# ARM-software/astc-encoder

Hardware: AMD Instinct MI355X
Metric: Mtexels/s + PSNR-dB, 8192x8192 RGBA8 LDR 6x6 -medium (higher is better)
Workload: dtype f32

## Files before the change

astc-encoder_amd/csrc/wave_partition.h:

```cpp
#pragma once
#include "wave_ctx.h"

namespace astcd { inline namespace ASTC_VARIANT {

struct PartScratch {
	uint64_t bitmaps[4];
	uint16_t mscount[64];
	int      best_count;
	int      best[MAX_PARTITIONING_CANDIDATES];
	int      n;
	int      lim;
	uint8_t  pad[256 - 32 - 128 - 4 - 32 - 8];
	WV_FN uint16_t* ordering() { return reinterpret_cast<uint16_t*>(reinterpret_cast<uint8_t*>(this) + 256); }
	WV_FN float* uncor_err() { return reinterpret_cast<float*>(reinterpret_cast<uint8_t*>(this) + 256 + n * 2); }
	WV_FN float* samec_err() { return uncor_err() + lim; }
	WV_FN uint8_t* mismatch() { return reinterpret_cast<uint8_t*>(samec_err() + lim); }
};
static_assert(sizeof(PartScratch) == 256, "PartScratch header");

WV_FN int mismatch2(const uint64_t* a, const uint64_t* b)
{
	int v1 = popcount64(a[0] ^ b[0]) + popcount64(a[1] ^ b[1]);
	int v2 = popcount64(a[0] ^ b[1]) + popcount64(a[1] ^ b[0]);
	return i_min(v1, v2) / 2;
}

WV_FN int mismatch3(const uint64_t* a, const uint64_t* b)
{
	int p00 = popcount64(a[0] ^ b[0]), p01 = popcount64(a[0] ^ b[1]), p02 = popcount64(a[0] ^ b[2]);
	int p10 = popcount64(a[1] ^ b[0]), p11 = popcount64(a[1] ^ b[1]), p12 = popcount64(a[1] ^ b[2]);
	int p20 = popcount64(a[2] ^ b[0]), p21 = popcount64(a[2] ^ b[1]), p22 = popcount64(a[2] ^ b[2]);
	int v0 = i_min(p11 + p22, p12 + p21) + p00;
	int v1 = i_min(p10 + p22, p12 + p20) + p01;
	int v2 = i_min(p10 + p21, p11 + p20) + p02;
	return i_min(i_min(v0, v1), v2) / 2;
}

WV_FN int mismatch4(const uint64_t* a, const uint64_t* b)
{
	int p[4][4];
	for (int i = 0; i < 4; i++) for (int j = 0; j < 4; j++) p[i][j] = popcount64(a[i] ^ b[j]);
	int mx23 = i_min(p[2][2] + p[3][3], p[2][3] + p[3][2]);
	int mx13 = i_min(p[2][1] + p[3][3], p[2][3] + p[3][1]);
	int mx12 = i_min(p[2][1] + p[3][2], p[2][2] + p[3][1]);
	int mx03 = i_min(p[2][0] + p[3][3], p[2][3] + p[3][0]);
	int mx02 = i_min(p[2][0] + p[3][2], p[2][2] + p[3][0]);
	int mx01 = i_min(p[2][1] + p[3][0], p[2][0] + p[3][1]);
	int v0 = p[0][0] + i_min(i_min(p[1][1] + mx23, p[1][2] + mx13), p[1][3] + mx12);
	int v1 = p[0][1] + i_min(i_min(p[1][0] + mx23, p[1][2] + mx03), p[1][3] + mx02);
	int v2 = p[0][2] + i_min(i_min(p[1][1] + mx03, p[1][0] + mx13), p[1][3] + mx01);
	int v3 = p[0][3] + i_min(i_min(p[1][1] + mx02, p[1][2] + mx01), p[1][0] + mx12);
	return i_min(i_min(v0, v1), i_min(v2, v3)) / 2;
}

WV_FN int kmeans_partition_ordering(const Ctx& c, int pc, PartScratch& ps)
{
	TrialInfo& tr = c.tr();
	const BlkInfo& blk = c.blk();
	const int T = c.T;
	float* dist = c.tsc_p(0);
	float* assign = c.tsc_p(1);
	const f4 cw = cw4_of(blk);
	float* centers = &tr.fbox[0];

	{
		int sample = 145897 % T;
		WV_ONE { for (int k = 0; k < 4; k++) centers[k] = c.data(k)[sample]; }
		WV_SYNC();
		int clusters_selected = 1;

		WV_FOR_T(i, T)
		{
			f4 color = mk4(c.data(0)[i], c.data(1)[i], c.data(2)[i], c.data(3)[i]);
			f4 diff = color - load4(centers);
			dist[i] = dot_s(diff * diff, cw);
		}
		WV_SYNC();

		const float cluster_cutoffs[9] = {
			0.626220f, 0.932770f, 0.275454f,
			0.318558f, 0.240113f, 0.009190f,
			0.347661f, 0.731960f, 0.156391f
		};
		int cutoff = (clusters_selected - 1) + 3 * (pc - 2);

		while (true)
		{
			float distance_sum = 0.0f;
			for (int i = 0; i < T; i++) distance_sum += dist[i];

			float summa = 0.0f;
			float distance_cutoff = distance_sum * cluster_cutoffs[cutoff++];
			sample = T;
			for (int i = 0; i < T; i++)
			{
				summa += dist[i];
				sample = (sample == T && summa >= distance_cutoff) ? i : sample;
			}
			sample = i_min(sample, T - 1);

			WV_SYNC();
			WV_ONE { for (int k = 0; k < 4; k++) centers[clusters_selected * 4 + k] = c.data(k)[sample]; }
			WV_SYNC();
			clusters_selected++;
			if (clusters_selected >= pc) break;

			WV_FOR_T(i, T)
			{
				f4 color = mk4(c.data(0)[i], c.data(1)[i], c.data(2)[i], c.data(3)[i]);
				f4 diff = color - load4(&centers[(clusters_selected - 1) * 4]);
				float distance = dot_s(diff * diff, cw);
				dist[i] = f_min(distance, dist[i]);
			}
			WV_SYNC();
		}
	}

	for (int iter = 0; iter < 3; iter++)
	{
		if (iter > 0)
		{
			WV_FOR64(k, pc * 4)
			{
				int p = k >> 2, ch = k & 3;
				const float* d = c.data(ch);
				float sum = 0.0f;
				int cnt = 0;
				for (int i = 0; i < T; i++)
				{
					const bool mine = (int)assign[i] == p;
					sum += mine ? d[i] : 0.0f;
					cnt += mine ? 1 : 0;
				}
				float scale = 1.0f / (float)cnt;
				tr.fbox[16 + k] = sum * scale;
			}
			WV_SYNC();
			WV_FOR64(k, pc * 4) { centers[k] = tr.fbox[16 + k]; }
			WV_SYNC();
		}

		WV_FOR_T(i, T)
		{
			float best_distance = 3.402823466e+38f;
			int best_partition = 0;
			f4 color = mk4(c.data(0)[i], c.data(1)[i], c.data(2)[i], c.data(3)[i]);
			for (int j = 0; j < pc; j++)
			{
				f4 diff = color - load4(&centers[j * 4]);
				float distance = dot_s(diff * diff, cw);
				if (distance < best_distance)
				{
					best_distance = distance;
					best_partition = j;
				}
			}
			assign[i] = (float)best_partition;
		}
		WV_SYNC();

		{
			int c0 = 0, c1 = 0, c2 = 0, c3 = 0;
#if WV_DEVICE
			for (int base = 0; base < T; base += 64)
			{
				const int i = base + WV_LANE;
				const int a = i < T ? (int)assign[i] : -1;
				c0 += __popcll(__ballot(a == 0)); c1 += __popcll(__ballot(a == 1));
				c2 += __popcll(__ballot(a == 2)); c3 += __popcll(__ballot(a == 3));
			}
#else
			for (int i = 0; i < T; i++)
			{
				int a = (int)assign[i];
				c0 += a == 0; c1 += a == 1; c2 += a == 2; c3 += a == 3;
			}
#endif
			bool any_empty = false;
			for (int i = 0; i < pc; i++) any_empty = any_empty || (i == 0 ? c0 : i == 1 ? c1 : i == 2 ? c2 : c3) == 0;
			if (any_empty)
			{
				WV_ONE
				{
					bool problem_case;
					do
					{
						problem_case = false;
						for (int i = 0; i < pc; i++)
						{
							int ci = i == 0 ? c0 : i == 1 ? c1 : i == 2 ? c2 : c3;
							if (ci == 0)
							{
								int a = (int)assign[i];
								c0 -= a == 0; c1 -= a == 1; c2 -= a == 2; c3 -= a == 3;
								c0 += i == 0; c1 += i == 1; c2 += i == 2; c3 += i == 3;
								assign[i] = (float)i;
								problem_case = true;
							}
						}
					} while (problem_case);
				}
				WV_SYNC();
			}
		}
	}

	const int texels_to_process = i_min(T, MAX_KMEANS_TEXELS);
	const uint8_t* km = c.table(c.root->off_kmeans_texels);
#if WV_DEVICE
	{
		const int a = WV_LANE < texels_to_process ? (int)assign[km[WV_LANE]] : -1;
		for (int p = 0; p < pc; p++)
		{
			const uint64_t bm = __ballot(a == p);
			WV_ONE { ps.bitmaps[p] = bm; }
		}
	}
#else
	WV_FOR64(p, pc)
	{
		uint64_t bm = 0;
		for (int i = 0; i < texels_to_process; i++)
		{
			if ((int)assign[km[i]] == p) bm |= 1ULL << i;
		}
		ps.bitmaps[p] = bm;
	}
#endif
	WV_SYNC();

	const int count = (int)c.root->partitioning_count_selected[pc - 1];
	const uint64_t* cov = reinterpret_cast<const uint64_t*>(c.table(c.root->off_coverage[pc - 1]));
	WV_FOR(i, count)
	{
		int m;
		if (pc == 2) m = mismatch2(ps.bitmaps, cov + i * 2);
		else if (pc == 3) m = mismatch3(ps.bitmaps, cov + i * 3);
		else m = mismatch4(ps.bitmaps, cov + i * 4);
		ps.mismatch()[i] = (uint8_t)m;
	}
	WV_SYNC();

#if WV_DEVICE
	{
		const int lane = WV_LANE;
		const uint8_t* mm = ps.mismatch();
		uint16_t* ord = ps.ordering();
		int* bins = &tr.ibox[0];
		bins[lane] = 0;
		WV_SYNC();
		auto same_key_lanes = [](int m, bool valid) -> unsigned long long
		{
			unsigned long long mask = __ballot(valid);
			#pragma unroll
			for (int k = 0; k < 6; k++)
			{
				const bool bit = ((m >> k) & 1) != 0;
				const unsigned long long with_bit = __ballot(bit);
				mask &= bit ? with_bit : ~with_bit;
			}
			return mask;
		};
		auto lanes_below = [](unsigned long long mask) -> int
		{
			return (int)__builtin_amdgcn_mbcnt_hi((uint32_t)(mask >> 32), __builtin_amdgcn_mbcnt_lo((uint32_t)mask, 0u));
		};
		for (int first = 0; first < count; first += 64)
		{
			const int i = first + lane;
			const bool valid = i < count;
			const int m = valid ? (int)mm[i] : 0;
			const unsigned long long same = same_key_lanes(m, valid);
			if (valid && lanes_below(same) == 0) bins[m] += (int)__popcll(same);
			WV_SYNC();
		}
		WV_SYNC();
		{
			const int hist = bins[lane];
			int base = hist;
			for (int d = 1; d < 64; d <<= 1)
			{
				int up = __shfl_up(base, d);
				if (lane >= d) base += up;
			}
			bins[lane] = base - hist;
		}
		WV_SYNC();
		for (int first = 0; first < count; first += 64)
		{
			const int i = first + lane;
			const bool valid = i < count;
			const int m = valid ? (int)mm[i] : 0;
			const unsigned long long same = same_key_lanes(m, valid);
			const int rank = lanes_below(same);
			const int start = bins[m];
			if (valid) ord[start + rank] = (uint16_t)i;
			if (valid && rank == 0) bins[m] = start + (int)__popcll(same);
			WV_SYNC();
		}
		(void)texels_to_process;
	}
#else
	WV_ONE
	{
		for (int i = 0; i < 64; i++) ps.mscount[i] = 0;
		for (int i = 0; i < count; i++) ps.mscount[ps.mismatch()[i]]++;
		uint16_t sum = 0;
		for (int i = 0; i < texels_to_process; i++)
		{
			uint16_t cnt = ps.mscount[i];
			ps.mscount[i] = sum;
			sum = (uint16_t)(sum + cnt);
		}
		for (int i = 0; i < count; i++)
		{
			unsigned int idx = ps.mscount[ps.mismatch()[i]]++;
			ps.ordering()[idx] = (uint16_t)i;
		}
	}
#endif
	WV_SYNC();
	return count;
}

template <bool USES_ALPHA>
WV_FN void score_partitioning(const Ctx& c, int pc, const PartView& pv, float weight_imprecision_estim, float& uncor_out, float& samec_out)
{
	const BlkInfo& blk = c.blk();
	const int T = c.T, Tp = c.Tp;
	constexpr int n = USES_ALPHA ? 4 : 3;

	float avg[4][4];
	{
		float rest[4];
		#pragma unroll
		for (int ch = 0; ch < 4; ch++) rest[ch] = blk.data_mean[ch] * (float)T;
		const uint32_t* ot4 = reinterpret_cast<const uint32_t*>(pv.of_texel);
		#pragma unroll
		for (int p = 0; p < 3; p++)
		{
			if (p >= pc - 1) break;
			float acc[4][4];
			#pragma unroll
			for (int ch = 0; ch < 4; ch++)
				#pragma unroll
				for (int l = 0; l < 4; l++) acc[ch][l] = 0.0f;
			#pragma nounroll
			for (int i = 0; i < Tp; i += 4)
			{
				const uint32_t ot = ot4[i >> 2];
				const float m0 = (int)(ot & 0xFF) == p ? 1.0f : 0.0f;
				const float m1 = (int)((ot >> 8) & 0xFF) == p ? 1.0f : 0.0f;
				const float m2 = (int)((ot >> 16) & 0xFF) == p ? 1.0f : 0.0f;
				const float m3 = (int)(ot >> 24) == p ? 1.0f : 0.0f;
				#pragma unroll
				for (int ch = 0; ch < 4; ch++)
				{
					if (ch >= n) break;
					const float* d = c.data(ch) + i;
					acc[ch][0] = f_add_masked(acc[ch][0], d[0], m0);
					acc[ch][1] = f_add_masked(acc[ch][1], d[1], m1);
					acc[ch][2] = f_add_masked(acc[ch][2], d[2], m2);
					acc[ch][3] = f_add_masked(acc[ch][3], d[3], m3);
				}
			}
			#pragma unroll
			for (int ch = 0; ch < 4; ch++)
			{
				if (ch >= n) break;
				float total = hadd4(acc[ch][0], acc[ch][1], acc[ch][2], acc[ch][3]);
				rest[ch] = rest[ch] - total;
				avg[p][ch] = total / (float)pv.cnt(p);
			}
			if (n == 3) avg[p][3] = 0.0f;
		}
		#pragma unroll
		for (int p = 1; p < 4; p++)
		{
			if (p != pc - 1) continue;
			#pragma unroll
			for (int ch = 0; ch < 4; ch++) avg[p][ch] = ch < n ? rest[ch] / (float)pv.cnt(p) : 0.0f;
		}
	}

	float ua0 = 0.0f, ua1 = 0.0f, ua2 = 0.0f, ua3 = 0.0f;
	float sa0 = 0.0f, sa1 = 0.0f, sa2 = 0.0f, sa3 = 0.0f;
	float tail_uncor[4], tail_samec[4];

	#pragma unroll
	for (int p = 0; p < 4; p++)
	{
		if (p >= pc) break;
		const uint8_t* tix = pv.sorted + pv.off(p);
		const int cnt = pv.cnt(p);
		f4 average = load4(avg[p]);

		f4 sum[4];
		#pragma unroll
		for (int k = 0; k < 4; k++) sum[k] = splat4(0.0f);
		for (int i = 0; i < cnt; i++)
		{
			int t = tix[i];
			f4 d = mk4(c.data(0)[t], c.data(1)[t], c.data(2)[t], n == 4 ? c.data(3)[t] : 0.0f) - average;
			auto add_masked4 = [](f4 acc, f4 v, float m) { return mk4(f_add_masked(acc.x, v.x, m), f_add_masked(acc.y, v.y, m), f_add_masked(acc.z, v.z, m), f_add_masked(acc.w, v.w, m)); };
			sum[0] = add_masked4(sum[0], d, d.x > 0.0f ? 1.0f : 0.0f);
			sum[1] = add_masked4(sum[1], d, d.y > 0.0f ? 1.0f : 0.0f);
			sum[2] = add_masked4(sum[2], d, d.z > 0.0f ? 1.0f : 0.0f);
			if (n == 4) sum[3] = add_masked4(sum[3], d, d.w > 0.0f ? 1.0f : 0.0f);
		}
		f4 best_vector = sum[0];
		float best_sum = dot_s(sum[0], sum[0]);
		#pragma unroll
		for (int k = 1; k < 4; k++)
		{
			if (k >= n) break;
			float prod = dot_s(sum[k], sum[k]);
			const bool better = prod > best_sum;
			best_vector = select4(better, sum[k], best_vector);
			best_sum = better ? prod : best_sum;
		}

		f4 ub = normalize_safe4(best_vector, n == 4 ? unit4() : unit3());
		f4 sb = normalize_safe4(average, n == 4 ? unit4() : unit3());
		float dd = n == 4 ? dot_s(average, ub) : dot3_s(average, ub);
		f4 amod = average - ub * (n == 4 ? splat4(dd) : mk4(dd, dd, dd, 0.0f));

		float lo = 1e10f, hi = -1e10f;
		auto one_texel = [&](int i, float& ua, float& sa)
		{
			int t = tix[i];
			float r = c.data(0)[t], g = c.data(1)[t], b = c.data(2)[t];
			float ue, se, uncor_param;
			if (n == 4)
			{
				float a = c.data(3)[t];
				uncor_param = (r * ub.x) + (g * ub.y) + (b * ub.z) + (a * ub.w);
				float d0 = (amod.x - r) + (uncor_param * ub.x);
				float d1 = (amod.y - g) + (uncor_param * ub.y);
				float d2 = (amod.z - b) + (uncor_param * ub.z);
				float d3 = (amod.w - a) + (uncor_param * ub.w);
				ue = (cw_of(blk, 0) * d0 * d0) + (cw_of(blk, 1) * d1 * d1) + (cw_of(blk, 2) * d2 * d2) + (cw_of(blk, 3) * d3 * d3);
				float sp = (r * sb.x) + (g * sb.y) + (b * sb.z) + (a * sb.w);
				float s0 = sp * sb.x - r, s1 = sp * sb.y - g, s2 = sp * sb.z - b, s3 = sp * sb.w - a;
				se = (cw_of(blk, 0) * s0 * s0) + (cw_of(blk, 1) * s1 * s1) + (cw_of(blk, 2) * s2 * s2) + (cw_of(blk, 3) * s3 * s3);
			}
			else
			{
				uncor_param = (r * ub.x) + (g * ub.y) + (b * ub.z);
				float d0 = (amod.x - r) + (uncor_param * ub.x);
				float d1 = (amod.y - g) + (uncor_param * ub.y);
				float d2 = (amod.z - b) + (uncor_param * ub.z);
				ue = (cw_of(blk, 0) * d0 * d0) + (cw_of(blk, 1) * d1 * d1) + (cw_of(blk, 2) * d2 * d2);
				float sp = (r * sb.x) + (g * sb.y) + (b * sb.z);
				float s0 = sp * sb.x - r, s1 = sp * sb.y - g, s2 = sp * sb.z - b;
				se = (cw_of(blk, 0) * s0 * s0) + (cw_of(blk, 1) * s1 * s1) + (cw_of(blk, 2) * s2 * s2);
			}
			lo = f_run_min(uncor_param, lo);
			hi = f_run_max(uncor_param, hi);
			ua += ue; sa += se;
		};
		for (int i = 0; i < cnt; i += 4)
		{
			one_texel(i, ua0, sa0);
			if (i + 1 < cnt) one_texel(i + 1, ua1, sa1);
			if (i + 2 < cnt) one_texel(i + 2, ua2, sa2);
			if (i + 3 < cnt) one_texel(i + 3, ua3, sa3);
		}
		float linelen = hi - lo;
		linelen = f_max(linelen, 1e-7f);
		{
			const f4 error_weights = splat4((float)cnt * weight_imprecision_estim);
			const f4 uncor_vector = ub * linelen;
			const f4 samec_vector = sb * linelen;
			if (n == 4)
			{
				tail_uncor[p] = dot_s(uncor_vector * uncor_vector, error_weights);
				tail_samec[p] = dot_s(samec_vector * samec_vector, error_weights);
			}
			else
			{
				tail_uncor[p] = dot3_s(uncor_vector * uncor_vector, error_weights);
				tail_samec[p] = dot3_s(samec_vector * samec_vector, error_weights);
			}
		}
	}

	float uncor_error = hadd4(ua0, ua1, ua2, ua3);
	float samec_error = hadd4(sa0, sa1, sa2, sa3);
	#pragma unroll
	for (int p = 0; p < 4; p++)
	{
		if (p >= pc) break;
		uncor_error += tail_uncor[p];
		samec_error += tail_samec[p];
	}
	uncor_out = uncor_error;
	samec_out = samec_error;
}

WV_FN void insert_result(int max_values, float this_error, int this_partition, float* best_errors, int* best_partitions)
{
	if (this_error >= best_errors[max_values - 1]) return;
	for (int i = 0; i < max_values; i++)
	{
		if (this_error > best_errors[i]) continue;
		for (int j = max_values - 1; j > i; j--)
		{
			best_errors[j] = best_errors[j - 1];
			best_partitions[j] = best_partitions[j - 1];
		}
		best_errors[i] = this_error;
		best_partitions[i] = this_partition;
		break;
	}
}


WV_FN int partition_search_order(const Ctx& c, int pc)
{
	PartScratch& ps = *reinterpret_cast<PartScratch*>(c.part());
	WV_ONE
	{
		uint32_t lim = c.cfg->tune_partition_index_limit[0];
		if (c.cfg->tune_partition_index_limit[1] > lim) lim = c.cfg->tune_partition_index_limit[1];
		if (c.cfg->tune_partition_index_limit[2] > lim) lim = c.cfg->tune_partition_index_limit[2];
		uint32_t n = (c.root->max_partitionings + 3u) & ~3u;
		ps.n = (int)n;
		ps.lim = (int)(lim < n ? lim : n);
	}
	WV_SYNC();
	return kmeans_partition_ordering(c, pc, ps);
}

WV_FN void partition_search_score(const Ctx& c, int pc, int partition_search_limit)
{
	WV_LANE_SCOPE;
	PartScratch& ps = *reinterpret_cast<PartScratch*>(c.part());
	const BlkInfo& blk = c.blk();
	const int T = c.T;
	float weight_imprecision_estim = 0.055f;
	if (T <= 20) weight_imprecision_estim = 0.03f;
	else if (T <= 31) weight_imprecision_estim = 0.04f;
	else if (T <= 41) weight_imprecision_estim = 0.05f;
	weight_imprecision_estim = wv_uniform(weight_imprecision_estim * weight_imprecision_estim);

	const bool uses_alpha = wv_uniform(!(blk.data_min[3] == blk.data_max[3]));

	{ PROF_SCOPE(c, PS_PSCORE);
	const int rec_words = wv_uniform((int)c.L->part_rec_words);
	const uint32_t rec_inv24 = wv_uniform(c.L->part_rec_inv24);
	const int chunk = wv_uniform((int)c.L->part_chunk);
	uint32_t* staged = reinterpret_cast<uint32_t*>(c.lds + c.L->part_tabs);
	const uint8_t* part_base = c.table(c.root->off_partitions[pc - 1]);
	const uint32_t part_stride = wv_uniform(c.root->partition_stride);
	for (int first = 0; first < partition_search_limit; first += chunk)
	{
		const int nn = i_min(chunk, partition_search_limit - first);
		WV_FOR(k, nn * rec_words)
		{
			int sl = (int)(((uint32_t)k * rec_inv24) >> 24), w = k - sl * rec_words;
			staged[wv_opaque(k)] = table_at_byte<uint32_t>(part_base, (uint32_t)ps.ordering()[first + sl] * part_stride + (uint32_t)w * 4u);
		}
		WV_SYNC();
		WV_FOR64(i_lane, nn)
		{
			const int i = wv_opaque(i_lane);
			const uint8_t* rec = reinterpret_cast<const uint8_t*>(staged + i * rec_words);
			PartView pv;
			pv.h = reinterpret_cast<const PartitionHeader*>(rec);
			pv.of_texel = rec + sizeof(PartitionHeader);
			pv.sorted = pv.of_texel + T;
			pv.pcount = pc;
			{
				uint32_t o = 0;
				pv.offsets = 0; pv.counts = 0;
				for (int q = 0; q < 4; q++)
				{
					uint32_t n = pv.h->texel_count[q];
					pv.offsets |= o << (8 * q); pv.counts |= n << (8 * q);
					o += n;
				}
			}
			float ue, se;
			if (uses_alpha) score_partitioning<true>(c, pc, pv, weight_imprecision_estim, ue, se);
			else score_partitioning<false>(c, pc, pv, weight_imprecision_estim, ue, se);
			ps.uncor_err()[first + i] = ue;
			ps.samec_err()[first + i] = se;
		}
		WV_SYNC();
	}
	}

}

WV_FN int partition_search_select(const Ctx& c, int partition_search_limit, int requested_candidates)
{
	PartScratch& ps = *reinterpret_cast<PartScratch*>(c.part());
#if WV_DEVICE
	if (partition_search_limit <= 64)
	{
		const int lane = WV_LANE;
		const bool live = lane < partition_search_limit;
		const float ue = live ? ps.uncor_err()[lane] : 0.0f;
		const float se = live ? ps.samec_err()[lane] : 0.0f;
		const int part = live ? (int)ps.ordering()[lane] : -1;
		int urank = 0, srank = 0;
		bool plain = !live || (ue < ERROR_CALC_DEFAULT && se < ERROR_CALC_DEFAULT);
		for (int j = 0; j < partition_search_limit; j++)
		{
			const float uj = int_as_float(__builtin_amdgcn_readlane(float_as_int(ue), j));
			const float sj = int_as_float(__builtin_amdgcn_readlane(float_as_int(se), j));
			urank += uj < ue ? 1 : 0;
			srank += sj < se ? 1 : 0;
			plain = plain && (j == lane || (uj != ue && sj != se));
		}
		if (__ballot(live && !plain) == 0ull)
		{
			int* slot_part = reinterpret_cast<int*>(ps.mscount);
			if (live && urank < requested_candidates) slot_part[2 * urank] = part;
			if (live && srank < requested_candidates) slot_part[2 * srank + 1] = part;
			WV_SYNC();
			const int nslots = 2 * requested_candidates;
			const int mine = lane < nslots ? slot_part[lane] : -1;
			bool repeat = false;
			for (int j = 0; j < nslots; j++)
			{
				const int pj = __builtin_amdgcn_readlane(mine, j);
				repeat = repeat || (j < lane && pj == mine);
			}
			const unsigned long long fresh = __ballot(lane < nslots && !repeat);
			const int at = __popcll(fresh & ((1ull << lane) - 1ull));
			if (lane < nslots && !repeat && at < requested_candidates) ps.best[at] = mine;
			const int emitted = i_min(__popcll(fresh), requested_candidates);
			WV_ONE { ps.best_count = emitted; }
			WV_SYNC();
			return emitted;
		}
	}
#endif
	WV_ONE
	{
		static_assert(sizeof(ps.mscount) >= 4 * MAX_PARTITIONING_CANDIDATES * 4, "top-N lists do not fit the sort bins");
		float* uncor_best_errors = reinterpret_cast<float*>(ps.mscount);
		float* samec_best_errors = uncor_best_errors + MAX_PARTITIONING_CANDIDATES;
		int* uncor_best_partitions = reinterpret_cast<int*>(samec_best_errors + MAX_PARTITIONING_CANDIDATES);
		int* samec_best_partitions = uncor_best_partitions + MAX_PARTITIONING_CANDIDATES;
		for (int i = 0; i < MAX_PARTITIONING_CANDIDATES; i++)
		{
			uncor_best_errors[i] = ERROR_CALC_DEFAULT; samec_best_errors[i] = ERROR_CALC_DEFAULT;
			uncor_best_partitions[i] = 0; samec_best_partitions[i] = 0;
		}
		for (int i = 0; i < partition_search_limit; i++)
		{
			int partition = ps.ordering()[i];
			insert_result(requested_candidates, ps.uncor_err()[i], partition, uncor_best_errors, uncor_best_partitions);
			insert_result(requested_candidates, ps.samec_err()[i], partition, samec_best_errors, samec_best_partitions);
		}

		int emitted = 0;
		for (int i = 0; i < requested_candidates * 2 && emitted < requested_candidates; i++)
		{
			int partition = (i & 1) ? samec_best_partitions[i >> 1] : uncor_best_partitions[i >> 1];
			bool written = false;
			for (int j = 0; j < emitted; j++) written = written || ps.best[j] == partition;
			if (!written) ps.best[emitted++] = partition;
		}
		ps.best_count = emitted;
	}
	WV_SYNC();
	return ps.best_count;
}

} }
```

Before: 238.7.

## Score partition candidates with lane quads sharing texel line-distance work

Restructures partition scoring on device so that each group of four lanes cooperates on one candidate's per-texel line-distance loop, instead of one lane walking every texel of its own candidate. Line parameters are exchanged through ds_bpermute, and min/max and error sums are reduced within each quad before being routed back to the owning lane. This is meant to cut the serial per-lane texel loop and the divergence caused by unequal partition sizes. In exchange it adds many cross-lane permutes, several passes when a chunk holds more than 16 candidates, and extra register arrays per pass.

```diff
diff --git a/astc-encoder_amd/csrc/wave_partition.h b/astc-encoder_amd/csrc/wave_partition.h
--- a/astc-encoder_amd/csrc/wave_partition.h
+++ b/astc-encoder_amd/csrc/wave_partition.h
@@ -1,5 +1,6 @@
 #pragma once
 #include "wave_ctx.h"
+#include "wave_quad.h"
 
 namespace astcd { inline namespace ASTC_VARIANT {
 
@@ -323,68 +324,119 @@
 	return count;
 }
 
+struct ScoreQuads {
+	const uint8_t* records;
+	int record_bytes;
+	int candidates;
+	int lane;
+};
+
+#if defined(ASTC_FIXED_CONTEXT)
+constexpr int kScorePasses = ((int)kFixedLayout.part_chunk + 15) / 16;
+#else
+constexpr int kScorePasses = 4;
+#endif
+
+template <int n>
+WV_FN void line_distance_texel(const Ctx& c, const BlkInfo& blk, int t, f4 ub, f4 sb, f4 amod, float& lo, float& hi, float& ua, float& sa)
+{
+	float r = c.data(0)[t], g = c.data(1)[t], b = c.data(2)[t];
+	float ue, se, uncor_param;
+	if (n == 4)
+	{
+		float a = c.data(3)[t];
+		uncor_param = (r * ub.x) + (g * ub.y) + (b * ub.z) + (a * ub.w);
+		float d0 = (amod.x - r) + (uncor_param * ub.x);
+		float d1 = (amod.y - g) + (uncor_param * ub.y);
+		float d2 = (amod.z - b) + (uncor_param * ub.z);
+		float d3 = (amod.w - a) + (uncor_param * ub.w);
+		ue = (cw_of(blk, 0) * d0 * d0) + (cw_of(blk, 1) * d1 * d1) + (cw_of(blk, 2) * d2 * d2) + (cw_of(blk, 3) * d3 * d3);
+		float sp = (r * sb.x) + (g * sb.y) + (b * sb.z) + (a * sb.w);
+		float s0 = sp * sb.x - r, s1 = sp * sb.y - g, s2 = sp * sb.z - b, s3 = sp * sb.w - a;
+		se = (cw_of(blk, 0) * s0 * s0) + (cw_of(blk, 1) * s1 * s1) + (cw_of(blk, 2) * s2 * s2) + (cw_of(blk, 3) * s3 * s3);
+	}
+	else
+	{
+		uncor_param = (r * ub.x) + (g * ub.y) + (b * ub.z);
+		float d0 = (amod.x - r) + (uncor_param * ub.x);
+		float d1 = (amod.y - g) + (uncor_param * ub.y);
+		float d2 = (amod.z - b) + (uncor_param * ub.z);
+		ue = (cw_of(blk, 0) * d0 * d0) + (cw_of(blk, 1) * d1 * d1) + (cw_of(blk, 2) * d2 * d2);
+		float sp = (r * sb.x) + (g * sb.y) + (b * sb.z);
+		float s0 = sp * sb.x - r, s1 = sp * sb.y - g, s2 = sp * sb.z - b;
+		se = (cw_of(blk, 0) * s0 * s0) + (cw_of(blk, 1) * s1 * s1) + (cw_of(blk, 2) * s2 * s2);
+	}
+	lo = f_run_min(uncor_param, lo);
+	hi = f_run_max(uncor_param, hi);
+	ua += ue; sa += se;
+}
+
 template <bool USES_ALPHA>
-WV_FN void score_partitioning(const Ctx& c, int pc, const PartView& pv, float weight_imprecision_estim, float& uncor_out, float& samec_out)
+WV_FN void score_partitioning(const Ctx& c, int pc, const PartView& pv, float weight_imprecision_estim, const ScoreQuads& sq, float& uncor_out, float& samec_out)
 {
 	const BlkInfo& blk = c.blk();
 	const int T = c.T, Tp = c.Tp;
 	constexpr int n = USES_ALPHA ? 4 : 3;
 
-	float avg[4][4];
-	{
-		float rest[4];
+	float rest[4];
+	#pragma unroll
+	for (int ch = 0; ch < 4; ch++) rest[ch] = blk.data_mean[ch] * (float)T;
+	auto partition_average = [&](int p, int cnt) -> f4
+	{
+		float av[4] = { 0.0f, 0.0f, 0.0f, 0.0f };
+		if (p == pc - 1)
+		{
+			#pragma unroll
+			for (int ch = 0; ch < n; ch++) av[ch] = rest[ch] / (float)cnt;
+			return load4(av);
+		}
+		const uint32_t* ot4 = reinterpret_cast<const uint32_t*>(pv.of_texel);
+		float acc[4][4];
 		#pragma unroll
-		for (int ch = 0; ch < 4; ch++) rest[ch] = blk.data_mean[ch] * (float)T;
-		const uint32_t* ot4 = reinterpret_cast<const uint32_t*>(pv.of_texel);
-		#pragma unroll
-		for (int p = 0; p < 3; p++)
-		{
-			if (p >= pc - 1) break;
-			float acc[4][4];
+		for (int ch = 0; ch < 4; ch++)
+			#pragma unroll
+			for (int l = 0; l < 4; l++) acc[ch][l] = 0.0f;
+		#pragma nounroll
+		for (int i = 0; i < Tp; i += 4)
+		{
+			const uint32_t ot = ot4[i >> 2];
+			const float m0 = (int)(ot & 0xFF) == p ? 1.0f : 0.0f;
+			const float m1 = (int)((ot >> 8) & 0xFF) == p ? 1.0f : 0.0f;
+			const float m2 = (int)((ot >> 16) & 0xFF) == p ? 1.0f : 0.0f;
+			const float m3 = (int)(ot >> 24) == p ? 1.0f : 0.0f;
 			#pragma unroll
 			for (int ch = 0; ch < 4; ch++)
-				#pragma unroll
-				for (int l = 0; l < 4; l++) acc[ch][l] = 0.0f;
-			#pragma nounroll
-			for (int i = 0; i < Tp; i += 4)
-			{
-				const uint32_t ot = ot4[i >> 2];
-				const float m0 = (int)(ot & 0xFF) == p ? 1.0f : 0.0f;
-				const float m1 = (int)((ot >> 8) & 0xFF) == p ? 1.0f : 0.0f;
-				const float m2 = (int)((ot >> 16) & 0xFF) == p ? 1.0f : 0.0f;
-				const float m3 = (int)(ot >> 24) == p ? 1.0f : 0.0f;
-				#pragma unroll
-				for (int ch = 0; ch < 4; ch++)
-				{
-					if (ch >= n) break;
-					const float* d = c.data(ch) + i;
-					acc[ch][0] = f_add_masked(acc[ch][0], d[0], m0);
-					acc[ch][1] = f_add_masked(acc[ch][1], d[1], m1);
-					acc[ch][2] = f_add_masked(acc[ch][2], d[2], m2);
-					acc[ch][3] = f_add_masked(acc[ch][3], d[3], m3);
-				}
-			}
-			#pragma unroll
-			for (int ch = 0; ch < 4; ch++)
 			{
 				if (ch >= n) break;
-				float total = hadd4(acc[ch][0], acc[ch][1], acc[ch][2], acc[ch][3]);
-				rest[ch] = rest[ch] - total;
-				avg[p][ch] = total / (float)pv.cnt(p);
-			}
-			if (n == 3) avg[p][3] = 0.0f;
+				const float* d = c.data(ch) + i;
+				acc[ch][0] = f_add_masked(acc[ch][0], d[0], m0);
+				acc[ch][1] = f_add_masked(acc[ch][1], d[1], m1);
+				acc[ch][2] = f_add_masked(acc[ch][2], d[2], m2);
+				acc[ch][3] = f_add_masked(acc[ch][3], d[3], m3);
+			}
 		}
 		#pragma unroll
-		for (int p = 1; p < 4; p++)
-		{
-			if (p != pc - 1) continue;
-			#pragma unroll
-			for (int ch = 0; ch < 4; ch++) avg[p][ch] = ch < n ? rest[ch] / (float)pv.cnt(p) : 0.0f;
-		}
-	}
-
+		for (int ch = 0; ch < 4; ch++)
+		{
+			if (ch >= n) break;
+			float total = hadd4(acc[ch][0], acc[ch][1], acc[ch][2], acc[ch][3]);
+			rest[ch] = rest[ch] - total;
+			av[ch] = total / (float)cnt;
+		}
+		return load4(av);
+	};
+
+#if WV_DEVICE
+	float uq[kScorePasses], sq_[kScorePasses];
+	#pragma unroll
+	for (int k = 0; k < kScorePasses; k++) { uq[k] = 0.0f; sq_[k] = 0.0f; }
+	const int lane = sq.lane;
+	const int back = (lane & 15) << 4;
+#else
+	(void)sq;
 	float ua0 = 0.0f, ua1 = 0.0f, ua2 = 0.0f, ua3 = 0.0f;
 	float sa0 = 0.0f, sa1 = 0.0f, sa2 = 0.0f, sa3 = 0.0f;
+#endif
 	float tail_uncor[4], tail_samec[4];
 
 	#pragma unroll
@@ -393,7 +445,7 @@
 		if (p >= pc) break;
 		const uint8_t* tix = pv.sorted + pv.off(p);
 		const int cnt = pv.cnt(p);
-		f4 average = load4(avg[p]);
+		f4 average = partition_average(p, cnt);
 
 		f4 sum[4];
 		#pragma unroll
@@ -425,68 +477,84 @@
 		float dd = n == 4 ? dot_s(average, ub) : dot3_s(average, ub);
 		f4 amod = average - ub * (n == 4 ? splat4(dd) : mk4(dd, dd, dd, 0.0f));
 
-		float lo = 1e10f, hi = -1e10f;
-		auto one_texel = [&](int i, float& ua, float& sa)
-		{
-			int t = tix[i];
-			float r = c.data(0)[t], g = c.data(1)[t], b = c.data(2)[t];
-			float ue, se, uncor_param;
+		auto tails = [&](f4 line_u, f4 line_s, float linelen, int texels, float& tail_u, float& tail_s)
+		{
+			const f4 error_weights = splat4((float)texels * weight_imprecision_estim);
+			const f4 uncor_vector = line_u * linelen;
+			const f4 samec_vector = line_s * linelen;
 			if (n == 4)
 			{
-				float a = c.data(3)[t];
-				uncor_param = (r * ub.x) + (g * ub.y) + (b * ub.z) + (a * ub.w);
-				float d0 = (amod.x - r) + (uncor_param * ub.x);
-				float d1 = (amod.y - g) + (uncor_param * ub.y);
-				float d2 = (amod.z - b) + (uncor_param * ub.z);
-				float d3 = (amod.w - a) + (uncor_param * ub.w);
-				ue = (cw_of(blk, 0) * d0 * d0) + (cw_of(blk, 1) * d1 * d1) + (cw_of(blk, 2) * d2 * d2) + (cw_of(blk, 3) * d3 * d3);
-				float sp = (r * sb.x) + (g * sb.y) + (b * sb.z) + (a * sb.w);
-				float s0 = sp * sb.x - r, s1 = sp * sb.y - g, s2 = sp * sb.z - b, s3 = sp * sb.w - a;
-				se = (cw_of(blk, 0) * s0 * s0) + (cw_of(blk, 1) * s1 * s1) + (cw_of(blk, 2) * s2 * s2) + (cw_of(blk, 3) * s3 * s3);
+				tail_u = dot_s(uncor_vector * uncor_vector, error_weights);
+				tail_s = dot_s(samec_vector * samec_vector, error_weights);
 			}
 			else
 			{
-				uncor_param = (r * ub.x) + (g * ub.y) + (b * ub.z);
-				float d0 = (amod.x - r) + (uncor_param * ub.x);
-				float d1 = (amod.y - g) + (uncor_param * ub.y);
-				float d2 = (amod.z - b) + (uncor_param * ub.z);
-				ue = (cw_of(blk, 0) * d0 * d0) + (cw_of(blk, 1) * d1 * d1) + (cw_of(blk, 2) * d2 * d2);
-				float sp = (r * sb.x) + (g * sb.y) + (b * sb.z);
-				float s0 = sp * sb.x - r, s1 = sp * sb.y - g, s2 = sp * sb.z - b;
-				se = (cw_of(blk, 0) * s0 * s0) + (cw_of(blk, 1) * s1 * s1) + (cw_of(blk, 2) * s2 * s2);
-			}
-			lo = f_run_min(uncor_param, lo);
-			hi = f_run_max(uncor_param, hi);
-			ua += ue; sa += se;
+				tail_u = dot3_s(uncor_vector * uncor_vector, error_weights);
+				tail_s = dot3_s(samec_vector * samec_vector, error_weights);
+			}
 		};
-		for (int i = 0; i < cnt; i += 4)
-		{
-			one_texel(i, ua0, sa0);
-			if (i + 1 < cnt) one_texel(i + 1, ua1, sa1);
-			if (i + 2 < cnt) one_texel(i + 2, ua2, sa2);
-			if (i + 3 < cnt) one_texel(i + 3, ua3, sa3);
-		}
-		float linelen = hi - lo;
-		linelen = f_max(linelen, 1e-7f);
-		{
-			const f4 error_weights = splat4((float)cnt * weight_imprecision_estim);
-			const f4 uncor_vector = ub * linelen;
-			const f4 samec_vector = sb * linelen;
-			if (n == 4)
-			{
-				tail_uncor[p] = dot_s(uncor_vector * uncor_vector, error_weights);
-				tail_samec[p] = dot_s(samec_vector * samec_vector, error_weights);
-			}
-			else
-			{
-				tail_uncor[p] = dot3_s(uncor_vector * uncor_vector, error_weights);
-				tail_samec[p] = dot3_s(samec_vector * samec_vector, error_weights);
-			}
-		}
-	}
-
+#if WV_DEVICE
+		{
+			const int mine_run = pv.off(p) | (cnt << 8);
+			tail_uncor[p] = 0.0f; tail_samec[p] = 0.0f;
+			for (int pass = 0; pass * 16 < sq.candidates; pass++)
+			{
+				const int src = pass * 16 + (lane >> 2);
+				const int from = src << 2;
+				auto take = [from](float v) { return int_as_float(__builtin_amdgcn_ds_bpermute(from, float_as_int(v))); };
+				const f4 qub = mk4(take(ub.x), take(ub.y), take(ub.z), n == 4 ? take(ub.w) : 0.0f);
+				const f4 qsb = mk4(take(sb.x), take(sb.y), take(sb.z), n == 4 ? take(sb.w) : 0.0f);
+				const f4 qamod = mk4(take(amod.x), take(amod.y), take(amod.z), n == 4 ? take(amod.w) : 0.0f);
+				const int run = __builtin_amdgcn_ds_bpermute(from, mine_run);
+				const int qcnt = src < sq.candidates ? run >> 8 : 0;
+				const uint8_t* qtix = sq.records + src * sq.record_bytes + (int)sizeof(PartitionHeader) + T + (run & 0xFF);
+				float ua = uq[0], sa = sq_[0];
+				#pragma unroll
+				for (int k = 1; k < kScorePasses; k++) { ua = pass == k ? uq[k] : ua; sa = pass == k ? sq_[k] : sa; }
+				float lo = 1e10f, hi = -1e10f;
+				for (int i = lane & 3; i < qcnt; i += 4) line_distance_texel<n>(c, blk, qtix[i], qub, qsb, qamod, lo, hi, ua, sa);
+				#pragma unroll
+				for (int k = 0; k < kScorePasses; k++) { uq[k] = pass == k ? ua : uq[k]; sq_[k] = pass == k ? sa : sq_[k]; }
+				qf qlo, qhi; qlo.v = lo; qhi.v = hi;
+				float tu, ts;
+				tails(qub, qsb, f_max(q_hmax(qhi) - q_hmin(qlo), 1e-7f), run >> 8, tu, ts);
+				tu = int_as_float(__builtin_amdgcn_ds_bpermute(back, float_as_int(tu)));
+				ts = int_as_float(__builtin_amdgcn_ds_bpermute(back, float_as_int(ts)));
+				tail_uncor[p] = (lane >> 4) == pass ? tu : tail_uncor[p];
+				tail_samec[p] = (lane >> 4) == pass ? ts : tail_samec[p];
+			}
+		}
+#else
+		{
+			float lo = 1e10f, hi = -1e10f;
+			for (int i = 0; i < cnt; i += 4)
+			{
+				line_distance_texel<n>(c, blk, tix[i], ub, sb, amod, lo, hi, ua0, sa0);
+				if (i + 1 < cnt) line_distance_texel<n>(c, blk, tix[i + 1], ub, sb, amod, lo, hi, ua1, sa1);
+				if (i + 2 < cnt) line_distance_texel<n>(c, blk, tix[i + 2], ub, sb, amod, lo, hi, ua2, sa2);
+				if (i + 3 < cnt) line_distance_texel<n>(c, blk, tix[i + 3], ub, sb, amod, lo, hi, ua3, sa3);
+			}
+			tails(ub, sb, f_max(hi - lo, 1e-7f), cnt, tail_uncor[p], tail_samec[p]);
+		}
+#endif
+	}
+
+#if WV_DEVICE
+	float uncor_error = 0.0f, samec_error = 0.0f;
+	#pragma unroll
+	for (int pass = 0; pass < kScorePasses; pass++)
+	{
+		if (pass * 16 >= sq.candidates) break;
+		qf qu, qs; qu.v = uq[pass]; qs.v = sq_[pass];
+		const float hu = int_as_float(__builtin_amdgcn_ds_bpermute(back, float_as_int(q_hadd(qu))));
+		const float hs = int_as_float(__builtin_amdgcn_ds_bpermute(back, float_as_int(q_hadd(qs))));
+		uncor_error = (lane >> 4) == pass ? hu : uncor_error;
+		samec_error = (lane >> 4) == pass ? hs : samec_error;
+	}
+#else
 	float uncor_error = hadd4(ua0, ua1, ua2, ua3);
 	float samec_error = hadd4(sa0, sa1, sa2, sa3);
+#endif
 	#pragma unroll
 	for (int p = 0; p < 4; p++)
 	{
@@ -562,7 +630,7 @@
 			staged[wv_opaque(k)] = table_at_byte<uint32_t>(part_base, (uint32_t)ps.ordering()[first + sl] * part_stride + (uint32_t)w * 4u);
 		}
 		WV_SYNC();
-		WV_FOR64(i_lane, nn)
+		auto score_candidate = [&](int i_lane, bool live, int lane)
 		{
 			const int i = wv_opaque(i_lane);
 			const uint8_t* rec = reinterpret_cast<const uint8_t*>(staged + i * rec_words);
@@ -581,12 +649,25 @@
 					o += n;
 				}
 			}
+			ScoreQuads sq;
+			sq.records = reinterpret_cast<const uint8_t*>(staged);
+			sq.record_bytes = rec_words * 4;
+			sq.candidates = nn;
+			sq.lane = lane;
 			float ue, se;
-			if (uses_alpha) score_partitioning<true>(c, pc, pv, weight_imprecision_estim, ue, se);
-			else score_partitioning<false>(c, pc, pv, weight_imprecision_estim, ue, se);
-			ps.uncor_err()[first + i] = ue;
-			ps.samec_err()[first + i] = se;
-		}
+			if (uses_alpha) score_partitioning<true>(c, pc, pv, weight_imprecision_estim, sq, ue, se);
+			else score_partitioning<false>(c, pc, pv, weight_imprecision_estim, sq, ue, se);
+			if (live)
+			{
+				ps.uncor_err()[first + i] = ue;
+				ps.samec_err()[first + i] = se;
+			}
+		};
+#if WV_DEVICE
+		score_candidate(i_min(WV_LANE, nn - 1), WV_LANE < nn, WV_LANE);
+#else
+		WV_FOR64(i_lane, nn) score_candidate(i_lane, true, 0);
+#endif
 		WV_SYNC();
 	}
 	}
```

Result: no change. 240.4, median of 6 (+0.7%).
